# rasmusab/bayes.js

Measured on NVIDIA B200. Metric: posterior draws/sec (chains x iters) Normal(mu,sigma) N=1024 at 1/2/4/8 B200, higher is better.
Workload: dtype f64

## Files before the change

### bayes.js_b200/csrc/amwg_jit.cuh

```cuda
#pragma once
#include <dlfcn.h>
#include <map>
#include <mutex>
#include <sstream>

namespace jit {

struct Insn {
  int pc = 0, next = 0;
  int op = 0, a = 0;
  bool acc = false, store = false;
  int mode[4] = {AMWG_MODE_NONE, AMWG_MODE_NONE, AMWG_MODE_NONE, AMWG_MODE_NONE};
  int inl[4] = {-1, -1, -1, -1};
  int extra[3] = {0, 0, 0};
  int n_extra = 0;
  int term = -1;
  int pops = 0, pushes = 0;
};

static bool has_result(int op) {
  switch (op) {
    case AMWG_OP_ACC: case AMWG_OP_ACC_RANGE: case AMWG_OP_PLATE: case AMWG_OP_LOOP_BEGIN: case AMWG_OP_LOOP_END:
    case AMWG_OP_STORE: case AMWG_OP_END: return false;
    default: return true;
  }
}

static bool decode(const amwg_model* md, int pc, Insn& in, std::string& err) {
  const int32_t* code = md->code;
  const int n = md->n_code;
  auto need = [&](int k) { if (pc + k > n) { err = "program runs past the end of the code"; return false; } return true; };
  in = Insn();
  in.pc = pc;
  if (!need(1)) return false;
  const unsigned w = (unsigned)code[pc++];
  in.op = (int)(w & 0xff);
  in.acc = (w >> 16) & 1;
  in.store = (w & AMWG_STORE_FLAG) != 0;
  in.a = (int)(w >> 18);
  if (in.op < 0 || in.op >= AMWG_OP__COUNT) { err = "unknown opcode"; return false; }
  int used[4] = {0, 0, 0, 0};
  if (in.op == AMWG_OP_PLATE) {
    if (in.a >= md->n_plates) { err = "plate index out of range"; return false; }
    const int kind = md->plates[in.a].kind;
    if (kind == AMWG_PLATE_NORM_IID) { used[0] = used[1] = 1; }
    else if (kind == AMWG_PLATE_BERN_IID || kind == AMWG_PLATE_NORM_GROUPED) { used[0] = 1; }
  } else {
    for (int k = 0; k < 4; ++k) used[k] = ((w >> (8 + 2 * k)) & 3) != AMWG_MODE_NONE;
  }
  for (int k = 3; k >= 0; --k) {
    if (!used[k]) continue;
    const int m = (w >> (8 + 2 * k)) & 3;
    in.mode[k] = m;
    if (m == AMWG_MODE_STACK) in.pops++;
    else if (m == AMWG_MODE_NONE) { err = "plate operand without a mode"; return false; }
    else { if (!need(1)) return false; in.inl[k] = code[pc++]; }
  }
  auto take = [&](int k) { if (!need(k)) return false; for (int j = 0; j < k; ++j) in.extra[in.n_extra++] = code[pc++]; return true; };
  switch (in.op) {
    case AMWG_OP_DATA: if (!take(1)) return false; break;
    case AMWG_OP_DATA_I: if (!take(2)) return false; break;
    case AMWG_OP_COMP_I: if (!take(3)) return false; break;
    case AMWG_OP_PLATE_SS: case AMWG_OP_ACC_RANGE: case AMWG_OP_LOOP_BEGIN: if (!take(1)) return false; break;
    case AMWG_OP_LOOP_END: if (!take(1)) return false; in.pops++; break;
    case AMWG_OP_ACC: case AMWG_OP_STORE: in.pops++; break;
    default: break;
  }
  if (has_result(in.op)) {
    if (in.acc) { if (in.store) { if (!need(1)) return false; in.term = code[pc++]; } }
    else in.pushes = 1;
  } else if (in.op == AMWG_OP_PLATE && in.store) {
    if (!need(1)) return false;
    in.term = code[pc++];
  }
  in.next = pc;
  return true;
}

static bool decode_program(const amwg_model* md, int pc, std::vector<Insn>& out, int* max_depth, std::string& err) {
  out.clear();
  int depth = 0, deepest = 0;
  if (pc < 0 || pc >= md->n_code) { err = "program offset out of range"; return false; }
  for (int guard = 0; guard < md->n_code + 1; ++guard) {
    Insn in;
    if (!decode(md, pc, in, err)) return false;
    depth -= in.pops;
    if (depth < 0) { err = "operand stack underflow"; return false; }
    depth += in.pushes;
    deepest = std::max(deepest, depth);
    out.push_back(in);
    if (in.op == AMWG_OP_END) { if (max_depth) *max_depth = deepest; return true; }
    pc = in.next;
  }
  err = "program has no END";
  return false;
}

static std::string lit(double v) {
  if (v != v) return "CUDART_NAN";
  if (v == INFINITY) return "CUDART_INF";
  if (v == -INFINITY) return "(-CUDART_INF)";
  char buf[64];
  snprintf(buf, sizeof buf, "%a", v);
  std::string s(buf);
  if (v < 0 || (v == 0 && std::signbit(v))) s = "(" + s + ")";
  return s;
}
static std::string istr(long long v) { return std::to_string(v); }
static std::string bits(double v) {
  long long b;
  memcpy(&b, &v, 8);
  return std::to_string(b) + "LL";
}

struct Plan {
  int threads = 128, minblocks = 7;
  int n_res = 0;
  std::vector<int> res_col, res_off, res_bytes;
  std::vector<int> col_smem_off;
  int stream_col = -1;
  int ring_off = 0, ring_stages = 4, ring_tile = 1024;
  int ws_smem = 0, ws_off = 0;
  unsigned smem_bytes = 0;
  std::vector<int> bern_mask_off;
};

struct Source {
  bool full = false;
  std::string generated;
  std::string prelude;
  Plan plan;
};

static const int kMaxGeneratedInsns = 6000;
static const unsigned kResidentBudget = 64u * 1024u;
static const unsigned kJitWsSmemLimit = 20u * 1024u;

struct Emitter {
  std::ostringstream os;
  std::map<std::string, std::string> cse;
  std::vector<std::string> stk;
  std::vector<std::map<std::string, std::string>> scopes;
  int nv = 0;
  std::string tmp(const std::string& rhs) {
    auto it = cse.find(rhs);
    if (it != cse.end()) return it->second;
    std::string name = "v" + std::to_string(nv++);
    os << "    const double " << name << " = " << rhs << ";\n";
    cse[rhs] = name;
    return name;
  }
};

struct Inst {
  std::vector<Insn> ins;
  int moved = -1;
// ... 228 lines not shown
        has_r = false;
        break;
      }
      case AMWG_OP_END: has_r = false; break;
      default: why = "opcode " + std::to_string(in.op) + " cannot be specialised"; return false;
    }
    if (!has_r) continue;
    std::string name = em.tmp(r);
    if (in.acc && cx == CTX_FULL) {
      em.os << "    lp = lp + " << name << ";\n";
    } else if (in.acc) {
      if (!in.store) { why = "a term of the sum is not cached"; return false; }
      terms.push_back(Term{gc.field(gather(i, [](const Insn& q) { return q.term; }), ix), name});
    } else {
      em.stk.push_back(name);
    }
  }
  return true;
}

static std::string insn_sig(const Insn& in) {
  char b[64];
  snprintf(b, sizeof b, "%d:%d%d%d%d:%d%d;", in.op, in.mode[0], in.mode[1], in.mode[2], in.mode[3], (int)in.acc, (int)in.store);
  return b;
}

static bool emit_step_class(const GenCtx& gc, const std::vector<Inst>& members, std::string& body, std::string& commit, int* n_insns, std::string& why) {
  const auto& rep = members[0].ins;
  std::vector<std::pair<size_t, size_t>> chunks;
  {
    size_t b0 = 0;
    for (size_t i = 0; i < rep.size(); ++i)
      if (rep[i].acc || rep[i].op == AMWG_OP_END) { chunks.emplace_back(b0, i + 1); b0 = i + 1; }
    if (b0 < rep.size()) chunks.emplace_back(b0, rep.size());
  }
  auto chunk_sig = [&](const std::pair<size_t, size_t>& ch) { std::string sg; for (size_t i = ch.first; i < ch.second; ++i) sg += insn_sig(rep[i]); return sg; };
  Emitter em;
  std::ostringstream bd, cm;
  std::vector<std::pair<int, std::string>> der;
  size_t k = 0;
  while (k < chunks.size()) {
    size_t run = 1;
    if (members.size() == 1 && rep[chunks[k].second - 1].acc) {
      const std::string sg = chunk_sig(chunks[k]);
      while (k + run < chunks.size() && chunk_sig(chunks[k + run]) == sg) ++run;
    }
    {
      std::vector<Term> terms; std::vector<std::string> cands;
      const size_t before = em.os.str().size();
      if (!emit_range(gc, members, chunks[k].first, chunks[k].second, "m", CTX_STEP, em, terms, cands, der, why)) return false;
      if (!em.stk.empty() && rep[chunks[k].second - 1].acc) { why = "a term leaves operands on the stack"; return false; }
      bd << em.os.str().substr(before);
      for (auto& t : terms) { bd << "    dl = dl + (" << t.val << " - TV(" << t.tid << "));\n"; cm << "    TV(" << t.tid << ") = " << t.val << ";\n"; }
      for (auto& sl : cands) cm << "    TV(" << sl << ") = TC(" << sl << ");\n";
      *n_insns += (int)(chunks[k].second - chunks[k].first);
    }
    if (run >= 4) {
      std::vector<Inst> iters;
      for (size_t j = 1; j < run; ++j) {
        Inst it;
        it.ins.assign(rep.begin() + chunks[k + j].first, rep.begin() + chunks[k + j].second);
        it.moved = members[0].moved;
        iters.push_back(it);
      }
      Emitter inner;
      inner.cse = em.cse;
      inner.nv = em.nv;
      std::vector<Term> terms; std::vector<std::string> cands;
      if (!emit_range(gc, iters, 0, iters[0].ins.size(), "j", CTX_STEP, inner, terms, cands, der, why)) return false;
      if (!inner.stk.empty()) { why = "a term leaves operands on the stack"; return false; }
      em.nv = inner.nv;
      bd << "    for (int j = 0; j < " << iters.size() << "; ++j) {\n" << inner.os.str();
      for (auto& t : terms) bd << "      dl = dl + (" << t.val << " - TV(" << t.tid << "));\n";
      bd << "    }\n";
      cm << "    for (int j = 0; j < " << iters.size() << "; ++j) {\n" << inner.os.str();
      for (auto& t : terms) cm << "      TV(" << t.tid << ") = " << t.val << ";\n";
      for (auto& sl : cands) cm << "      TV(" << sl << ") = TC(" << sl << ");\n";
      cm << "    }\n";
      *n_insns += (int)iters[0].ins.size();
      k += run;
    } else {
      k += 1;
    }
  }
  body = bd.str();
  commit = cm.str();
  return true;
}

static std::string signature(const std::vector<Insn>& prog) {
  std::string s;
  for (const Insn& in : prog) {
    char b[64];
    snprintf(b, sizeof b, "%d:%d%d%d%d:%d%d;", in.op, in.mode[0], in.mode[1], in.mode[2], in.mode[3], (int)in.acc, (int)in.store);
    s += b;
  }
  return s;
}

static std::string choose_shape(Plan& pl, unsigned off, size_t per_thread, unsigned long long n_chains, int sm_count) {
  const unsigned base = off;
  int best_t = 0, best_r = 1, best_ws = 0;
  double best_eff = -1.0;
  const int cands[] = {128, 64, 96, 160, 192, 224, 256};
  int forced_t = 0;
  if (const char* e = getenv("AMWG_JIT_THREADS")) { int t = atoi(e); if (t >= 32 && t <= 1024 && t % 32 == 0) forced_t = t; }
  for (int t : cands) {
    if (forced_t) t = forced_t;
    const size_t need = pad16(per_thread * (size_t)t);
    const int ws_smem = need <= kJitWsSmemLimit;
    const unsigned smem = std::max((unsigned)(pad16(base) + (ws_smem ? need : 0)), 16u);
    int r_max = (int)std::min<unsigned>(std::min<unsigned>((227u * 1024u) / (smem + 1024u), 2048u / (unsigned)t), 8u);
    if (r_max < 1) continue;
    const double ctas = std::ceil((double)n_chains / t);
    const double cap = (double)sm_count * r_max;
    double eff; int r_need;
    if (ctas <= cap) { const double per_sm = std::ceil(ctas / sm_count); eff = ((double)n_chains / sm_count) / (per_sm * t); r_need = (int)per_sm; }
    else { eff = ctas / (std::ceil(ctas / cap) * cap) * ((double)n_chains / (ctas * t)); r_need = r_max; }
    if (eff > best_eff + (best_t == 0 ? 0.0 : 0.15)) { best_eff = eff; best_t = t; best_r = r_need; best_ws = ws_smem; }
    if (forced_t) break;
  }
  if (!best_t) return "no launch shape fits";
  pl.threads = best_t;
  if (best_ws) { pl.ws_smem = 1; pl.ws_off = (int)pad16(off); off = (unsigned)(pad16(off) + pad16(per_thread * (size_t)best_t)); }
  pl.smem_bytes = std::max(off, 16u);
  pl.minblocks = std::max(1, best_r);
  if (const char* e = getenv("AMWG_JIT_MINBLOCKS")) { int v = atoi(e); if (v >= 1 && v <= 16) pl.minblocks = v; }
  return "";
}


static void emit_param_tables(std::ostringstream& tables, const amwg_model* md) {
  const int P = md->n_params;
  auto ptab = [&](const char* ty, const char* name, auto get) {
    tables << "__constant__ " << ty << " " << name << "[" << P << "] = {";
    for (int p = 0; p < P; ++p) tables << (p ? "," : "") << get(md->params[p]);
    tables << "};\n";
  };
  ptab("int", "JP_TYPE", [](const amwg_param& p) { return istr(p.type); });
  ptab("int", "JP_NCOMP", [](const amwg_param& p) { return istr(p.n_comp); });
  ptab("int", "JP_DIM0", [](const amwg_param& p) { return istr(p.dim0); });
  ptab("int", "JP_OFF", [](const amwg_param& p) { return istr(p.comp_offset); });
  ptab("long long", "JP_LOWER", [](const amwg_param& p) { return bits(p.lower); });
  ptab("long long", "JP_UPPER", [](const amwg_param& p) { return bits(p.upper); });
  tables << "__device__ __forceinline__ int jp_type(int p) { return JP_TYPE[p]; }\n"
            "__device__ __forceinline__ int jp_ncomp(int p) { return JP_NCOMP[p]; }\n"
            "__device__ __forceinline__ int jp_dim0(int p) { return JP_DIM0[p]; }\n"
            "__device__ __forceinline__ int jp_off(int p) { return JP_OFF[p]; }\n"
            "__device__ __forceinline__ double jp_lower(int p) { return __longlong_as_double(JP_LOWER[p]); }\n"
            "__device__ __forceinline__ double jp_upper(int p) { return __longlong_as_double(JP_UPPER[p]); }\n";
}


static std::string build_source(const amwg_model* md, const std::vector<double>& consts, unsigned long long n_chains, int sm_count,
                                double norm_c0, Source& src) {
  if (!md->comp_prog || md->n_terms <= 0 || md->stat_prog < 0) return "the model has no pre-evaluated statistics";
  if (md->n_variant_comps > 0) return "variant programs";
  const int D = md->n_comp, P = md->n_params, NT = md->n_terms;
  if (D > 65535 || P > 255) return "too many components / parameters";
  int max_dim0 = 1;
  for (int p = 0; p < P; ++p) {
    if (md->params[p].type == AMWG_BINARY) return "binary parameter";
    if (md->params[p].n_comp > 1) max_dim0 = std::max(max_dim0, std::max(md->params[p].dim0, 2));
  }
  std::string err;

  std::vector<Insn> stat;
  if (!decode_program(md, md->stat_prog, stat, nullptr, err)) return "stat_prog: " + err;
  struct StatEntry { int q, slot, comp; size_t first, last; bool simple; };
  std::vector<StatEntry> entries;
  {
    size_t start = 0;
    for (size_t i = 0; i < stat.size(); ++i) {
      if (stat[i].op == AMWG_OP_END) break;
      if (stat[i].op != AMWG_OP_PLATE_SS) continue;
      StatEntry e{stat[i].a, stat[i].extra[0], -1, start, i, false};
      if (e.q < 0 || e.q >= md->n_plates || md->plates[e.q].kind != AMWG_PLATE_NORM_IID) return "stat_prog refers to a plate that is not NORM_IID";
      if (e.slot < 0 || e.slot >= NT) return "statistic slot out of range";
      if (i == start && stat[i].mode[0] == AMWG_MODE_COMP) { e.simple = true; e.comp = stat[i].inl[0]; if (e.comp < 0 || e.comp >= D) return "component out of range"; }
      entries.push_back(e);
      start = i + 1;
    }
  }
  if (entries.empty()) return "no plate statistics";

  Plan& pl = src.plan;
  pl = Plan();
  pl.col_smem_off.assign(md->n_columns, -1);
  std::vector<char> col_used(md->n_columns, 0);
  for (const auto& e : entries) {
    const int c = md->plates[e.q].col[0];
    if (c < 0 || c >= md->n_columns) return "plate column out of range";
    const amwg_plate& p = md->plates[e.q];
    if (p.iparam[2] < 0 || (long long)p.iparam[2] + p.n > md->columns[c].n) return "plate runs past its column";
    col_used[c] = 1;
  }
  unsigned off = 0;
  std::vector<int> big;
  for (int c = 0; c < md->n_columns; ++c) {
    if (!col_used[c]) continue;
    const unsigned bytes = pad16(std::max<size_t>(sizeof(double) * (size_t)md->columns[c].n, 16));
    if (off + bytes <= kResidentBudget) {
      pl.col_smem_off[c] = (int)off; pl.res_col.push_back(c); pl.res_off.push_back((int)off); pl.res_bytes.push_back((int)bytes);
      off += bytes;
    } else big.push_back(c);
  }
  pl.n_res = (int)pl.res_col.size();
  if (big.size() > 1) return "more than one column exceeds shared memory";
  std::vector<StatEntry> r_entries, s_entries, x_entries;
  for (const auto& e : entries) {
    const int c = md->plates[e.q].col[0];
    const bool resident = pl.col_smem_off[c] >= 0;
    if (e.simple) (resident ? r_entries : s_entries).push_back(e);
    else { if (!resident) return "a plate with an expression mean lies on a streamed column"; x_entries.push_back(e); }
  }
  int s_begin = 0, s_total = 0;
  if (!big.empty()) {
    pl.stream_col = big[0];
    if (s_entries.empty()) return "streamed column without plates";
    std::stable_sort(s_entries.begin(), s_entries.end(), [&](const StatEntry& a, const StatEntry& b) { return md->plates[a.q].iparam[2] < md->plates[b.q].iparam[2]; });
    s_begin = md->plates[s_entries[0].q].iparam[2];
    if (s_begin & 1) return "streamed plates start at an odd offset";
    int cur = s_begin;
    for (const auto& e : s_entries) {
      const amwg_plate& p = md->plates[e.q];
      if (p.iparam[2] != cur || p.n <= 0) return "streamed plates do not tile their column";
      cur += p.n;
    }
    s_total = cur - s_begin;
    pl.ring_off = (int)off;
    off += (unsigned)(pl.ring_stages * pl.ring_tile * 8);
  }
  {
    const size_t per_thread = sizeof(double) * (size_t)(2 * NT + 3 * D) + sizeof(unsigned short) * (size_t)D;
    std::string e = choose_shape(pl, off, per_thread, n_chains, sm_count);
    if (!e.empty()) return e;
  }

  std::ostringstream tables, funcs;
  int table_counter = 0;
  GenCtx gc;
  gc.md = md; gc.consts = &consts; gc.tables = &tables; gc.table_counter = &table_counter;
  std::vector<std::vector<Insn>> progs(D);
  std::map<std::string, std::vector<int>> classes_by_sig;
  std::vector<std::string> sig_order;
  int total_insns = 0;
  for (int c = 0; c < D; ++c) {
    std::vector<Insn> full;
    if (!decode_program(md, md->comp_prog[c], full, nullptr, err)) return "comp_prog: " + err;
    for (const Insn& in : full) if (in.op != AMWG_OP_ACC_RANGE) progs[c].push_back(in);
    std::string sg = signature(progs[c]);
    if (!classes_by_sig.count(sg)) sig_order.push_back(sg);
    classes_by_sig[sg].push_back(c);
  }
  std::vector<int> cls_of(D, 0), mem_of(D, 0);
  funcs << "namespace amwg {\n";
  std::ostringstream step;
  step << "__device__ __forceinline__ bool jit_step(const int c, const double prop, const double coin, double* __restrict__ wk, const unsigned long long ws,\n"
          "                                         double* __restrict__ sp, const unsigned long long ss) {\n";
  if (sig_order.size() > 1) step << "  switch (JCLS[c]) {\n";
  bool need_mem = false;
  for (size_t k = 0; k < sig_order.size(); ++k) {
    const std::vector<int>& members = classes_by_sig[sig_order[k]];
    std::vector<Inst> inst;
    for (size_t m = 0; m < members.size(); ++m) {
      Inst it; it.ins = progs[members[m]]; it.moved = members[m];
      inst.push_back(it);
      cls_of[members[m]] = (int)k; mem_of[members[m]] = (int)m;
    }
    std::string body, commit, why;
    if (!emit_step_class(gc, inst, body, commit, &total_insns, why)) return "component program: " + why;
    if (total_insns > kMaxGeneratedInsns) return "the component programs are too long to specialise";
    if (commit.empty()) return "a component touches no term";
    if (sig_order.size() > 1) step << "  case " << k << ": {\n";
    else step << "  {\n";
    if (inst.size() > 1) { step << "    const int m = JMEM[c];\n"; need_mem = true; }
    step << "    double dl = 0.0;\n" << body;
    step << "    if (!(js_exp(dl) > coin)) return false;            // Metropolis accept (mcmc.js:527-534): strict >, NaN rejects\n";
    step << "    ST(c) = prop;\n" << commit;
    step << "    return true;\n  }\n";
  }
  if (sig_order.size() > 1) step << "  }\n  return false;\n";
  step << "}\n";

  std::ostringstream extra;
  extra << "__device__ __forceinline__ void jit_stat_extra(unsigned char* smem, double* __restrict__ wk, const unsigned long long ws,\n"
           "                                               double* __restrict__ sp, const unsigned long long ss, const bool wr) {\n";
  for (const auto& e : x_entries) {
    Inst it;
    it.ins.assign(stat.begin() + e.first, stat.begin() + e.last);
    std::vector<Inst> inst{it};
    const Insn pss = stat[e.last];
    Emitter em;
    std::vector<Term> terms; std::vector<std::string> cands; std::vector<std::pair<int, std::string>> der;
    std::string why;
    if (!emit_range(gc, inst, 0, it.ins.size(), "m", CTX_STAT, em, terms, cands, der, why)) return "stat_prog: " + why;
    std::string mean;
    if (pss.mode[0] == AMWG_MODE_STACK) { if (em.stk.empty()) return "stat_prog: missing mean"; mean = em.stk.back(); }
    else if (pss.mode[0] == AMWG_MODE_CONST) { if (pss.inl[0] < 0 || pss.inl[0] >= md->n_consts) return "stat_prog: const out of range"; mean = lit(consts[pss.inl[0]]); }
    else mean = "BP(" + std::to_string(pss.inl[0]) + ")";
    total_insns += (int)it.ins.size();
    const amwg_plate& p = md->plates[e.q];
    const int so = pl.col_smem_off[p.col[0]] + 8 * p.iparam[2];
    extra << "  {\n" << em.os.str();
    extra << "    const double S = sum_sq_dev(reinterpret_cast<const double*>(smem + " << so << "), smem_u32(smem) + " << so << "u, " << p.n << ", " << mean << ");\n";
    extra << "    if (wr) TC(" << e.slot << ") = S;\n  }\n";
  }
  extra << "  (void)smem; (void)wk; (void)ws; (void)sp; (void)ss; (void)wr;\n}\n";

  std::ostringstream dfun;
  if (md->n_derived > 0) {
    Inst it;
    if (!decode_program(md, md->derived_prog, it.ins, nullptr, err)) return "derived_prog: " + err;
    std::vector<Inst> inst{it};
    Emitter em;
    std::vector<Term> terms; std::vector<std::string> cands; std::vector<std::pair<int, std::string>> der;
    std::string why;
    if (!emit_range(gc, inst, 0, it.ins.size(), "m", CTX_DERIVED, em, terms, cands, der, why)) return "derived program: " + why;
    dfun << "__device__ __forceinline__ void jit_derived(const double* __restrict__ sp, const unsigned long long ss, double* der) {\n" << em.os.str();
    for (auto& d : der) { if (d.first < 0 || d.first >= md->n_derived) return "derived index out of range"; dfun << "    der[" << d.first << "] = " << d.second << ";\n"; }
    dfun << "}\n";
  }

  auto int_table = [&](const char* qual, const char* name, const std::vector<long long>& v) {
    tables << qual << " " << name << "[" << std::max<size_t>(v.size(), 1) << "] = {";
    for (size_t i = 0; i < v.size(); ++i) tables << (i ? "," : "") << v[i];
    if (v.empty()) tables << "0";
    tables << "};\n";
  };
  {
    std::vector<long long> v;
    if (sig_order.size() > 1) { v.assign(cls_of.begin(), cls_of.end()); int_table("__device__ const unsigned char", "JCLS", v); }
    if (need_mem) { v.assign(mem_of.begin(), mem_of.end()); int_table("__device__ const unsigned short", "JMEM", v); }
    tables << "__device__ const long long KCB[" << std::max(md->n_consts, 1) << "] = {";
    for (int i = 0; i < md->n_consts; ++i) tables << (i ? "," : "") << bits(consts[i]);
    if (md->n_consts == 0) tables << "0LL";
    tables << "};\n#define KC(i) __longlong_as_double(KCB[i])\n";
    emit_param_tables(tables, md);
    std::vector<long long> a, b, c2, d;
    for (int k = 0; k < pl.n_res; ++k) { a.push_back(pl.res_off[k]); b.push_back(pl.res_col[k]); c2.push_back(pl.res_bytes[k]); }
    int_table("__constant__ unsigned", "JRES_OFF", a); int_table("__constant__ int", "JRES_COL", b); int_table("__constant__ unsigned", "JRES_BYTES", c2);
    a.clear(); b.clear(); c2.clear();
    for (const auto& e : r_entries) {
      const amwg_plate& p = md->plates[e.q];
      a.push_back(e.comp); b.push_back(pl.col_smem_off[p.col[0]] + 8 * p.iparam[2]); c2.push_back(p.n); d.push_back(e.slot);
    }
    int_table("__constant__ int", "JR_COMP", a); int_table("__constant__ unsigned", "JR_SOFF", b); int_table("__constant__ int", "JR_N", c2); int_table("__constant__ int", "JR_SLOT", d);
    a.clear(); b.clear(); d.clear();
    int cur = 0;
    for (const auto& e : s_entries) { cur += md->plates[e.q].n; a.push_back(e.comp); b.push_back(cur); d.push_back(e.slot); }
    int_table("__constant__ int", "JS_COMP", a); int_table("__constant__ int", "JS_END", b); int_table("__constant__ int", "JS_SLOT", d);
  }

  unsigned long long res_total = 0;
  for (int k = 0; k < pl.n_res; ++k) res_total += (unsigned)pl.res_bytes[k];
  int jblock = -1;
  for (int p = 0, best = 7; p < P; ++p) {
    const amwg_param& pa = md->params[p];
    if (pa.n_comp <= best) continue;
    bool indep = true;
    std::vector<int> owner((size_t)NT, -1);
    for (int c = pa.comp_offset; c < pa.comp_offset + pa.n_comp && indep; ++c)
      for (int k = md->touch_off[c]; k < md->touch_off[c + 1]; ++k) {
        int& o = owner[(size_t)md->touch_terms[k]];
        if (o >= 0 && o != c) { indep = false; break; }
        o = c;
      }
    if (indep) { jblock = p; best = pa.n_comp; }
  }
  if (const char* e = getenv("AMWG_JIT_BLOCK")) { if (atoi(e) == 0) jblock = -1; }
  const bool jblock_free = jblock >= 0 && md->params[jblock].lower == -INFINITY && md->params[jblock].upper == INFINITY;
  std::ostringstream pre;
  pre << "#define JBLOCK " << jblock << "\n#define JBLOCK_FREE " << (jblock_free ? 1 : 0) << "\n";
  pre << "#define JD " << D << "\n#define JP " << P << "\n#define JNT " << NT << "\n#define JNSUM " << md->n_sum_terms << "\n"
      << "#define JTHREADS " << pl.threads << "\n#define JMINB " << pl.minblocks << "\n#define JWS_SMEM " << pl.ws_smem << "\n#define JWS_OFF " << pl.ws_off << "\n"
      << "#define JN_DERIVED " << md->n_derived << "\n#define JMAX_DIM0 " << max_dim0 << "\n#define JMAXCOL " << kMaxColumns << "\n"
      << "#define JN_RES " << pl.n_res << "\n#define JRES_TOTAL_BYTES " << res_total << "u\n#define JN_RSTAT " << r_entries.size() << "\n"
      << "#define JSTREAM " << (pl.stream_col >= 0 ? 1 : 0) << "\n#define JS_COL " << std::max(pl.stream_col, 0) << "\n#define JS_BEGIN " << s_begin << "\n#define JS_TOTAL " << s_total << "\n"
      << "#define JN_SSTAT " << s_entries.size() << "\n#define JRING_OFF " << pl.ring_off << "u\n#define JRING_STAGES " << pl.ring_stages << "\n#define JRING_TILE " << pl.ring_tile << "\n"
      << "#define JNORM_C0 " << lit(norm_c0) << "\n#define AMWG_REAL 0\n#define AMWG_INT 1\n#define AMWG_BINARY 2\n";
  int nacc = 4;
  if (const char* e = getenv("AMWG_JIT_NACC")) { int v = atoi(e); if (v == 4 || v == 8) nacc = v; }
  pre << "#define AMWG_NACC " << nacc << "\n";

  src.prelude = pre.str();
  funcs << tables.str() << step.str() << extra.str() << dfun.str() << "}  // namespace amwg\n";
  src.generated = funcs.str();
  return "";
}


static std::string build_source_full(const amwg_model* md, const std::vector<double>& consts, unsigned long long n_chains, int sm_count,
                                     double norm_c0, Source& src) {
  if (md->comp_prog && md->n_terms > 0) return "the model steps with a term cache";
  const int D = md->n_comp, P = md->n_params;
  if (D > 65535 || P > 255) return "too many components / parameters";
  int max_dim0 = 1;
  for (int p = 0; p < P; ++p) if (md->params[p].n_comp > 1) max_dim0 = std::max(max_dim0, std::max(md->params[p].dim0, 2));
  std::string err;
  Plan& pl = src.plan;
  pl = Plan();
  pl.col_smem_off.assign(md->n_columns, -1);
  unsigned off = 0;
  for (int c = 0; c < md->n_columns; ++c) {
    const unsigned bytes = pad16(std::max<size_t>(sizeof(double) * (size_t)md->columns[c].n, 16));
    if (off + bytes > kResidentBudget) return "the data does not fit in shared memory";
    pl.col_smem_off[c] = (int)off; pl.res_col.push_back(c); pl.res_off.push_back((int)off); pl.res_bytes.push_back((int)bytes);
    off += bytes;
  }
  pl.n_res = (int)pl.res_col.size();
  pl.bern_mask_off.assign(std::max(md->n_plates, 0), -1);
  std::vector<long long> bm_plate;
  for (int q = 0; q < md->n_plates; ++q) {
    const amwg_plate& pq = md->plates[q];
    if (pq.kind != AMWG_PLATE_BERN_IID || pq.n < 1 || pq.col[0] < 0 || pq.col[0] >= md->n_columns) continue;
    if (pq.iparam[2] < 0 || (long long)pq.iparam[2] + pq.n > md->columns[pq.col[0]].n) return "a plate runs past its column";
    off = (unsigned)pad16(off);
    pl.bern_mask_off[q] = (int)off; bm_plate.push_back(q);
    off += 4u * (unsigned)((pq.n + 31) / 32 + 1);
  }
  { std::string e = choose_shape(pl, off, sizeof(double) * (size_t)D, n_chains, sm_count); if (!e.empty()) return e; }

  std::ostringstream tables, funcs;
  int table_counter = 0, total_insns = 0;
  GenCtx gc;
  gc.md = md; gc.consts = &consts; gc.tables = &tables; gc.table_counter = &table_counter; gc.plan = &pl;
  const int n_var = md->n_variant_comps ? (1 << md->n_variant_comps) : 1;
  auto emit_program = [&](int pc, const std::string& name, bool derived) -> std::string {
    Inst it;
    if (!decode_program(md, pc, it.ins, nullptr, err)) return "program: " + err;
    total_insns += (int)it.ins.size();
    if (total_insns > kMaxGeneratedInsns) return "the programs are too long to specialise";
    std::vector<Inst> inst{it};
    Emitter em;
    std::vector<Term> terms; std::vector<std::string> cands; std::vector<std::pair<int, std::string>> der;
    std::string why;
// ... 215 lines not shown
```

### bayes.js_b200/csrc/amwg_jit_kernel.cuh

```cuda
#pragma once

namespace amwg {

struct JitArgs {
  ChainArrays a;
  SweepArgs sa;
  const double* col[JMAXCOL];
  const unsigned char* adapting;
};

#define TV(t) wk[(unsigned long long)(t) * ws]
#define TC(t) wk[(unsigned long long)(JNT + (t)) * ws]
#define BP(c) wk[(unsigned long long)(2 * JNT + (c)) * ws]
#define BC(c) wk[(unsigned long long)(2 * JNT + JD + (c)) * ws]
#define ST(c) sp[(unsigned long long)(c) * ss]

}

#include "amwg_jit_generated.inc"

namespace amwg {

extern "C" __global__ void __launch_bounds__(JTHREADS, JMINB) amwg_jit_sweep(const __grid_constant__ JitArgs A) {
  extern __shared__ __align__(16) unsigned char smem[];
  __shared__ __align__(8) unsigned long long bar_res;
#if JSTREAM
  __shared__ __align__(8) unsigned long long ring_full[JRING_STAGES];
#endif
  const ChainArrays& a = A.a;
  const SweepArgs& sa = A.sa;
  const unsigned long long C = a.C;
  const unsigned long long tid = (unsigned long long)blockIdx.x * blockDim.x + threadIdx.x;
  const bool valid = tid < C;
  const unsigned long long chain = valid ? tid : C - 1;
  const unsigned long long gchain = a.first_chain + chain;

  if (threadIdx.x == 0) {
    mbar_init(&bar_res, 1);
#if JSTREAM
    for (int k = 0; k < JRING_STAGES; ++k) mbar_init(&ring_full[k], 1);
#endif
    asm volatile("fence.mbarrier_init.release.cluster;" ::: "memory");
  }
  __syncthreads();
#if JN_RES > 0
  if (threadIdx.x == 0) {
    mbar_expect_tx(&bar_res, JRES_TOTAL_BYTES);
#pragma unroll
    for (int k = 0; k < JN_RES; ++k) tma_bulk_g2s(smem + JRES_OFF[k], A.col[JRES_COL[k]], JRES_BYTES[k], &bar_res);
  }
  mbar_wait(&bar_res, 0);
#endif

#if JWS_SMEM
  double* wk = reinterpret_cast<double*>(smem + JWS_OFF) + threadIdx.x;
  const unsigned long long ws = JTHREADS, ss = JTHREADS;
  double* sp = wk + (unsigned long long)(2 * JNT + 2 * JD) * ws;
  unsigned short* vq = reinterpret_cast<unsigned short*>(smem + JWS_OFF + (size_t)(2 * JNT + 3 * JD) * JTHREADS * sizeof(double)) + threadIdx.x;
  for (int t = 0; t < JNT; ++t) TV(t) = a.tval[(unsigned long long)t * C + chain];
  for (int c = 0; c < JD; ++c) ST(c) = a.state[(unsigned long long)c * C + chain];
  const bool wr = true;
#else
  double* wk = a.tval + chain;
  const unsigned long long ws = C, ss = C;
  double* sp = a.state + chain;
  unsigned short* vq = a.vseq + chain;
  const bool wr = valid;
#endif

  RandomStream g;
  g.init(a.rng_n[chain]);
  unsigned long long perm = a.perm[chain];
#if JMAX_DIM0 > 1
  unsigned char order[JMAX_DIM0 < kLocalOrder ? JMAX_DIM0 : kLocalOrder];
#endif
#if JSTREAM
  unsigned ring_fills = 0;
#endif

  long long rec_phase = sa.record ? sa.sample_i0 % sa.thin : 0;
  long long row = sa.record ? (sa.sample_i0 + sa.thin - 1) / sa.thin : 0;
  for (long long s = 0; s < sa.n_sweeps; ++s) {
    if (sa.record) {
      const bool rec_now = rec_phase == 0;
      if (++rec_phase == sa.thin) rec_phase = 0;
      if (rec_now && valid) {
#if JN_DERIVED > 0
        double der[JN_DERIVED];
        bool have_der = false;
#endif
        for (int j = 0; j < sa.n_monitor; ++j) {
          const int e = sa.monitor[j];
          double v;
          if (e < JD) {
            v = ST(e);
          } else {
#if JN_DERIVED > 0
            if (!have_der) { jit_derived(sp, ss, der); have_der = true; }
            v = der[e - JD];
#else
            v = CUDART_NAN;
#endif
          }
          sa.out[((unsigned long long)row * sa.n_monitor + j) * C + chain] = v;
        }
      }
      if (rec_now) ++row;
    }
#if JP > 1
    for (int i = JP - 1; i > 0; --i) {
      const int j = (int)floor(g.next(a.seed, gchain) * (i + 1));
      perm_swap(a, perm, chain, i, j, valid);
    }
#endif
    int pos = 0;
#pragma unroll 1
    for (int slot = 0; slot < JP; ++slot) {
      const int p = (JP > 1) ? perm_get(a, perm, chain, slot) : 0;
      const int n_comp = jp_ncomp(p), off = jp_off(p), ptype = jp_type(p);
      const double lower = jp_lower(p), upper = jp_upper(p);
#if JMAX_DIM0 > 1
      const int dim0 = jp_dim0(p);
      const int inner = n_comp / dim0;
      if (n_comp > 1) {
        for (int i = 0; i < dim0; ++i) ord_set(a, order, chain, dim0, i, i, valid);
        for (int i = dim0 - 1; i > 0; --i) {
          const int j = (int)floor(g.next(a.seed, gchain) * (i + 1));
          const int t = ord_get(a, order, chain, dim0, i);
          ord_set(a, order, chain, dim0, i, ord_get(a, order, chain, dim0, j), valid);
          ord_set(a, order, chain, dim0, j, t, valid);
        }
      }
#endif
#pragma unroll 1
      for (int r = 0; r < n_comp; ++r, ++pos) {
        int c = off;
#if JMAX_DIM0 > 1
        if (n_comp > 1) c += ord_get(a, order, chain, dim0, r / inner) * inner + (r % inner);
#endif
#if JBLOCK >= 0 && JBLOCK_FREE
        if (p == JBLOCK) {
          const double z = js_rnorm_ratio(g, a.seed, gchain);
          const double coin = g.next(a.seed, gchain);
          if (wr) { BP(c) = z; BC(c) = coin; }
          continue;
        }
#endif
        const double cur = ST(c);
        double prop = js_rnorm(g, a.seed, gchain, cur, a.psd[(unsigned long long)c * C + chain]);
        if (ptype == AMWG_INT) prop = js_round(prop);
        const bool inb = !(prop < lower || prop > upper);
        const double coin = inb ? g.next(a.seed, gchain) : -1.0;
        if (wr) {
          BP(c) = inb ? prop : cur;
          BC(c) = coin;
          vq[(unsigned long long)pos * ws] = (unsigned short)c;
        }
      }
    }
#if JBLOCK >= 0 && JBLOCK_FREE
    {
      const int n_b = jp_ncomp(JBLOCK), off_b = jp_off(JBLOCK);
      const bool is_int = jp_type(JBLOCK) == AMWG_INT;
#pragma unroll 4
      for (int r = 0; r < n_b; ++r) {
        const int c = off_b + r;
        double prop = BP(c) * a.psd[(unsigned long long)c * C + chain] + ST(c);
        if (is_int) prop = js_round(prop);
// ... 139 lines not shown
```

Before: 4.569 billion.

## Screen Metropolis accept with fp32 estimate and merge step classes around shared transcendentals

Adds an accept screen that decides the Metropolis test from the sign of dl or an fp32 exp2 estimate with a safety margin, falling back to the f64 exp only when undecided. It also rewrites multi-class component steps so that each class's independent log/exp calls are hoisted into shared slots evaluated once outside the class switch, which reduces warp divergence on expensive transcendentals. Both paths are on by default through environment flags. The merge relies on regex parsing of generated code, which could be brittle, and the screen adds branches and fp32 work on every step.

```diff
diff --git a/bayes.js_b200/csrc/amwg_jit.cuh b/bayes.js_b200/csrc/amwg_jit.cuh
--- a/bayes.js_b200/csrc/amwg_jit.cuh
+++ b/bayes.js_b200/csrc/amwg_jit.cuh
@@ -1,7 +1,10 @@
 #pragma once
 #include <dlfcn.h>
+#include <array>
 #include <map>
 #include <mutex>
+#include <regex>
+#include <set>
 #include <sstream>
 
 namespace jit {
@@ -536,6 +539,130 @@
 }
 
 
+static bool env_flag(const char* name, bool dflt) {
+  const char* e = getenv(name);
+  return e ? atoi(e) != 0 : dflt;
+}
+
+struct StepClass { std::string body, commit; bool uses_m; };
+
+static bool emit_merged_step(const std::vector<StepClass>& cls, const std::string& accept_test, std::ostringstream& out) {
+  static const std::regex def_re("^    const double (v[0-9]+) = (.*);$"), name_re("\\bv[0-9]+\\b");
+  static const char* const kHeavy[2] = {"js_log", "js_exp"};
+  auto refs_of = [](const std::string& s) {
+    std::set<std::string> r;
+    for (std::sregex_iterator it(s.begin(), s.end(), name_re), e; it != e; ++it) r.insert(it->str());
+    return r;
+  };
+  auto heavy_of = [](const std::string& rhs, std::string& arg) -> int {
+    for (int f = 0; f < 2; ++f) {
+      const std::string head = std::string(kHeavy[f]) + "(";
+      if (rhs.compare(0, head.size(), head) != 0 || rhs.back() != ')') continue;
+      int depth = 0;
+      for (size_t i = head.size() - 1; i < rhs.size(); ++i) {
+        depth += rhs[i] == '(' ? 1 : rhs[i] == ')' ? -1 : 0;
+        if (depth == 0 && i + 1 != rhs.size()) return -1;
+      }
+      arg = rhs.substr(head.size(), rhs.size() - head.size() - 1);
+      return f;
+    }
+    return -1;
+  };
+  struct Stmt { std::string text, name, rhs; bool def = false; int heavy = -1, slot = -1; std::string arg; bool phase_a = false; };
+  std::vector<std::vector<Stmt>> body(cls.size());
+  int n_slots[2] = {0, 0};
+  std::vector<std::array<std::vector<std::string>, 2>> args(cls.size());
+  bool uses_m = false;
+  for (size_t k = 0; k < cls.size(); ++k) {
+    uses_m = uses_m || cls[k].uses_m;
+    std::istringstream in(cls[k].body);
+    std::vector<Stmt>& st = body[k];
+    for (std::string ln; std::getline(in, ln);) {
+      Stmt s;
+      std::smatch mt;
+      if (ln.compare(0, 9, "    for (") == 0) {
+        s.text = ln + "\n";
+        bool closed = false;
+        while (!closed && std::getline(in, ln)) { s.text += ln + "\n"; closed = ln == "    }"; }
+        if (!closed) return false;
+      } else if (std::regex_match(ln, mt, def_re)) {
+        s.def = true; s.name = mt[1]; s.rhs = mt[2];
+      } else {
+        s.text = ln + "\n";
+      }
+      st.push_back(s);
+    }
+    std::set<std::string> tainted;
+    int used[2] = {0, 0};
+    for (Stmt& s : st) {
+      if (!s.def) continue;
+      bool dep = false;
+      for (const auto& r : refs_of(s.rhs)) dep = dep || tainted.count(r);
+      std::string arg;
+      const int f = heavy_of(s.rhs, arg);
+      if (f >= 0 && !dep) { s.heavy = f; s.slot = used[f]++; s.arg = arg; args[k][f].push_back(arg); }
+      if (f >= 0 || dep) tainted.insert(s.name);
+    }
+    for (int f = 0; f < 2; ++f) n_slots[f] = std::max(n_slots[f], used[f]);
+    std::set<std::string> need;
+    for (int f = 0; f < 2; ++f) for (const auto& a : args[k][f]) for (const auto& r : refs_of(a)) need.insert(r);
+    for (size_t i = st.size(); i-- > 0;)
+      if (st[i].def && st[i].heavy < 0 && need.count(st[i].name) && !tainted.count(st[i].name)) {
+        st[i].phase_a = true;
+        for (const auto& r : refs_of(st[i].rhs)) need.insert(r);
+      }
+  }
+  auto ren = [&](size_t k, const std::string& s) { return std::regex_replace(s, name_re, "k" + std::to_string(k) + "_$&"); };
+  auto slot_var = [](const char* pre, int f, int j) { return std::string(pre) + (f == 0 ? "l" : "e") + std::to_string(j); };
+  auto all_have = [&](int f, int j) { for (const auto& a : args) if ((int)a[f].size() <= j) return false; return true; };
+
+  out << "__device__ __forceinline__ bool jit_step(const int c, const double prop, const double coin, double* __restrict__ wk, const unsigned long long ws,\n"
+         "                                         double* __restrict__ sp, const unsigned long long ss) {\n";
+  if (uses_m) out << "  const int m = JMEM[c];\n";
+  for (size_t k = 0; k < cls.size(); ++k) {
+    std::string names;
+    for (const Stmt& s : body[k]) if (s.def) names += (names.empty() ? "" : ", ") + ren(k, s.name);
+    if (!names.empty()) out << "  double " << names << ";\n";
+  }
+  for (int f = 0; f < 2; ++f)
+    for (int j = 0; j < n_slots[f]; ++j) {
+      out << "  double " << slot_var("a", f, j) << " = 1.0;\n";
+      if (!all_have(f, j)) out << "  bool " << slot_var("u", f, j) << " = false;\n";
+    }
+  out << "  double dl = 0.0;\n  switch (JCLS[c]) {\n";
+  for (size_t k = 0; k < cls.size(); ++k) {
+    out << "  case " << k << ": {\n";
+    for (const Stmt& s : body[k]) if (s.phase_a) out << "    " << ren(k, s.name) << " = " << ren(k, s.rhs) << ";\n";
+    for (int f = 0; f < 2; ++f)
+      for (int j = 0; j < (int)args[k][f].size(); ++j) {
+        out << "    " << slot_var("a", f, j) << " = " << ren(k, args[k][f][j]) << ";\n";
+        if (!all_have(f, j)) out << "    " << slot_var("u", f, j) << " = true;\n";
+      }
+    out << "    break;\n  }\n";
+  }
+  out << "  }\n";
+  for (int f = 0; f < 2; ++f)
+    for (int j = 0; j < n_slots[f]; ++j) {
+      const std::string call = std::string(kHeavy[f]) + "(" + slot_var("a", f, j) + ")";
+      if (all_have(f, j)) out << "  const double " << slot_var("r", f, j) << " = " << call << ";\n";
+      else out << "  double " << slot_var("r", f, j) << " = 0.0;\n  if (" << slot_var("u", f, j) << ") " << slot_var("r", f, j) << " = " << call << ";\n";
+    }
+  out << "  switch (JCLS[c]) {\n";
+  for (size_t k = 0; k < cls.size(); ++k) {
+    out << "  case " << k << ": {\n";
+    for (const Stmt& s : body[k]) {
+      if (s.phase_a) continue;
+      if (!s.def) out << ren(k, s.text);
+      else out << "    " << ren(k, s.name) << " = " << (s.heavy >= 0 ? slot_var("r", s.heavy, s.slot) : ren(k, s.rhs)) << ";\n";
+    }
+    out << "    break;\n  }\n";
+  }
+  out << "  }\n" << accept_test << "  ST(c) = prop;\n  switch (JCLS[c]) {\n";
+  for (size_t k = 0; k < cls.size(); ++k) out << "  case " << k << ": {\n" << ren(k, cls[k].commit) << "    break;\n  }\n";
+  out << "  }\n  return true;\n}\n";
+  return true;
+}
+
 static std::string build_source(const amwg_model* md, const std::vector<double>& consts, unsigned long long n_chains, int sm_count,
                                 double norm_c0, Source& src) {
   if (!md->comp_prog || md->n_terms <= 0 || md->stat_prog < 0) return "the model has no pre-evaluated statistics";
@@ -639,6 +766,12 @@
   }
   std::vector<int> cls_of(D, 0), mem_of(D, 0);
   funcs << "namespace amwg {\n";
+  const bool screen = env_flag("AMWG_JIT_ACCEPT_SCREEN", true);
+  const std::string accept_test = screen ? "    int acc_ = jit_accept_screen(dl, coin);              // certain from dl's sign or an fp32 estimate; -1: undecided\n"
+                                           "    if (acc_ < 0) acc_ = js_exp(dl) > coin;            // Metropolis accept (mcmc.js:527-534): strict >, NaN rejects\n"
+                                           "    if (!acc_) return false;\n"
+                                         : "    if (!(js_exp(dl) > coin)) return false;            // Metropolis accept (mcmc.js:527-534): strict >, NaN rejects\n";
+  std::vector<StepClass> step_classes;
   std::ostringstream step;
   step << "__device__ __forceinline__ bool jit_step(const int c, const double prop, const double coin, double* __restrict__ wk, const unsigned long long ws,\n"
           "                                         double* __restrict__ sp, const unsigned long long ss) {\n";
@@ -660,12 +793,17 @@
     else step << "  {\n";
     if (inst.size() > 1) { step << "    const int m = JMEM[c];\n"; need_mem = true; }
     step << "    double dl = 0.0;\n" << body;
-    step << "    if (!(js_exp(dl) > coin)) return false;            // Metropolis accept (mcmc.js:527-534): strict >, NaN rejects\n";
+    step << accept_test;
     step << "    ST(c) = prop;\n" << commit;
     step << "    return true;\n  }\n";
+    step_classes.push_back(StepClass{body, commit, inst.size() > 1});
   }
   if (sig_order.size() > 1) step << "  }\n  return false;\n";
   step << "}\n";
+  if (sig_order.size() > 1 && env_flag("AMWG_JIT_MERGE_STEPS", true)) {
+    step.str("");
+    if (!emit_merged_step(step_classes, accept_test, step)) return "component program: unexpected generated step code";
+  }
 
   std::ostringstream extra;
   extra << "__device__ __forceinline__ void jit_stat_extra(unsigned char* smem, double* __restrict__ wk, const unsigned long long ws,\n"
diff --git a/bayes.js_b200/csrc/amwg_jit_kernel.cuh b/bayes.js_b200/csrc/amwg_jit_kernel.cuh
--- a/bayes.js_b200/csrc/amwg_jit_kernel.cuh
+++ b/bayes.js_b200/csrc/amwg_jit_kernel.cuh
@@ -14,6 +14,16 @@
 #define BP(c) wk[(unsigned long long)(2 * JNT + (c)) * ws]
 #define BC(c) wk[(unsigned long long)(2 * JNT + JD + (c)) * ws]
 #define ST(c) sp[(unsigned long long)(c) * ss]
+
+__device__ __forceinline__ int jit_accept_screen(const double dl, const double coin) {
+  if (dl >= 0.0) return 1;
+  if (!(coin > 0.0)) return -1;
+  if (dl < -40.0) return 0;
+  const double est = (double)exp2f((float)(dl * 1.4426950408889634));
+  if (est > coin * (1.0 + 0x1p-16)) return 1;
+  if (est < coin * (1.0 - 0x1p-16)) return 0;
+  return -1;
+}
 
 }
 
```

Measured after the change: 5.174 billion (median of 6 runs). 1.13x the previous value.
